# pmgbergen/porepy

Hardware: AMD Instinct MI355X
Metric: cells/sec MPFA assemble+solve, 3D unstructured grid (higher is better)
Workload: dtype f64

## Files before the change

include/porefv.h:

```cpp
#ifndef POREFV_H
#define POREFV_H

#include <stddef.h>
#include <stdint.h>

#ifdef __cplusplus
extern "C" {
#endif

typedef struct pfv_ctx pfv_ctx;

typedef enum {
  PFV_OK = 0,
  PFV_ERR_SINGULAR = 1,
  PFV_ERR_CELL_SHAPE = 2,
  PFV_ERR_HIP = 3,
  PFV_ERR_ARGUMENT = 4,
  PFV_ERR_UNSUPPORTED = 5,
  PFV_ERR_NOT_CONVERGED = 6
} pfv_status;

enum {
  PFV_MAT_FLUX = 0,
  PFV_MAT_BOUND_FLUX = 1,
// ... 401 lines not shown
pfv_status pfv_set_stream(pfv_ctx* h, void* hip_stream);
pfv_status pfv_reset_stream(pfv_ctx* h);
pfv_status pfv_sync(pfv_ctx* h);

pfv_status pfv_get_stats(pfv_ctx* h, pfv_stats* out);
pfv_status pfv_get_stats_n(pfv_ctx* h, void* out, size_t struct_size);

enum { PFV_KERNEL_SPMV_A = 0, PFV_KERNEL_NODE = 1, PFV_KERNEL_FACE = 2,
       PFV_KERNEL_AMG_SMOOTH = 3,
       PFV_KERNEL_TRIAD = 4,
       PFV_KERNEL_READ = 5         };
pfv_status pfv_time_kernel(pfv_ctx* h, int kernel, int reps, double* avg_ms);

pfv_status pfv_debug_copy(pfv_ctx* h, int which, double* dst, int64_t count);

#ifdef __cplusplus
}
#endif
#endif
```

porepy_amd/_lib.py:

```python
from __future__ import annotations

import ctypes as C
import os

import numpy as np

_HERE = os.path.dirname(os.path.abspath(__file__))
DEFAULT_LIBRARY = os.path.join(_HERE, "csrc", "libporefv_hip.so")

MAT_FLUX, MAT_BOUND_FLUX, MAT_BOUND_PRESSURE_CELL, MAT_BOUND_PRESSURE_FACE = 0, 1, 2, 3
MAT_VECTOR_SOURCE, MAT_BOUND_PRESSURE_VECTOR_SOURCE, MAT_SYSTEM = 4, 5, 6
MAT_STRESS, MAT_BOUND_STRESS, MAT_BOUND_DISPLACEMENT_CELL, MAT_BOUND_DISPLACEMENT_FACE, MAT_MECH_SYSTEM = 7, 8, 9, 10, 11
MAT_USER_SYSTEM = 12
MAT_FLUX_JACOBIAN = 13
MAT_UPWIND, MAT_UPWIND_RHS_DIR, MAT_UPWIND_RHS_NEU, MAT_TRANSPORT_SYSTEM = 14, 15, 16, 17
MAT_ADVDIFF_SYSTEM = 18
BC_DIR, BC_NEU, BC_ROB, BC_INTERNAL = 1, 2, 4, 8
SOLVE_CG, SOLVE_BICGSTAB, SOLVE_GMRES = 0, 1, 2
PRECOND_JACOBI, PRECOND_AMG, PRECOND_BLOCK, PRECOND_AMG_NNS, PRECOND_SWEEP = 0, 1, 2, 3, 4
FLUXFN_LINEAR, FLUXFN_COREY, FLUXFN_TABLE = 0, 1, 2
DISCR_REBUILD_TOPOLOGY, DISCR_SKIP_VECTOR_SOURCE = 1, 2

STATUS_NAMES = {
    0: "ok", 1: "singular local system", 2: "unsupported cell shape", 3: "HIP error",
# ... 8 lines not shown
    "pfv_spmv_device_rows", "pfv_copy_device_vector", "pfv_set_stream",
    "pfv_mpsa_set_params", "pfv_mpsa_discretize", "pfv_mpsa_assemble",
    "pfv_mpfa_discretize_faces", "pfv_set_system", "pfv_tpfa_discretize", "pfv_mpsa_discretize_faces", "pfv_set_preconditioner", "pfv_amg_setup", "pfv_amg_setup_sharded", "pfv_amg_apply_device", "pfv_csr_from_host", "pfv_csr_from_matrix", "pfv_csr_block_diag", "pfv_csr_matmul", "pfv_csr_axpby", "pfv_csr_transpose", "pfv_csr_bmat", "pfv_csr_scale", "pfv_csr_divide", "pfv_csr_spmv", "pfv_csr_spmv_device", "pfv_csr_info", "pfv_csr_get", "pfv_csr_set_system", "pfv_csr_free", "pfv_reset_stream", "pfv_mpsa_set_robin", "pfv_mpsa_set_basis", "pfv_mpfa_set_subface_bc", "pfv_mpsa_set_subface_bc", "pfv_mpsa_set_subface_basis",
    "pfv_biot_set_alphas", "pfv_biot_discretize", "pfv_biot_matrix_info", "pfv_biot_get_matrix",
    "pfv_set_vectors_on_device", "pfv_set_periodic", "pfv_biot_discretize_faces", "pfv_solve_sharded", "pfv_tpfa_transmissibility_ad",
    "pfv_get_matrix_rows", "pfv_active_size", "pfv_device_memory",
    "pfv_rccl_unique_id", "pfv_rccl_comm_create", "pfv_rccl_set_halo_plan", "pfv_rccl_hooks", "pfv_rccl_stats",
    "pfv_rccl_last_error", "pfv_rccl_comm_destroy", "pfv_mpfa_ad_flux_system", "pfv_host_alloc", "pfv_host_free",
    "pfv_mpsa_set_subface_eta", "pfv_mpsa_set_reconstruction_eta", "pfv_mpsa_set_reconstruction_eta_subface", "pfv_get_stats_n", "pfv_set_block_preconditioner",
    "pfv_mpfa_set_permeability", "pfv_set_near_null_space", "pfv_amg_nns_level", "pfv_amg_nns_apply_device", "pfv_amg_level",
    "pfv_mpfa_face_flux", "pfv_upwind_set_bc", "pfv_upwind_discretize", "pfv_upwind_assemble", "pfv_transport_advance",
    "pfv_advdiff_assemble", "pfv_advdiff_advance", "pfv_advdiff_face_flux", "pfv_resident_flux",
    "pfv_sweep_info", "pfv_transport_advance_multi", "pfv_transport_advance_nl", "pfv_transport_advance_nl_multi",
    "pfv_transport_advance_react", "pfv_transport_adjoint_multi", "pfv_transport_adjoint_react",
    "pfv_transport_adjoint_nl", "pfv_transport_adjoint_nl_multi", "pfv_flow_adjoint", "pfv_flow_adjoint_exact",
    "pfv_advdiff_adjoint", "pfv_advdiff_adjoint_exact", "pfv_amg_level_rhs",
]


class SolveInfo(C.Structure):
    _fields_ = [("iterations", C.c_int32), ("converged", C.c_int32),
                ("rel_residual", C.c_double), ("solve_ms", C.c_double)]


class Stats(C.Structure):
    _fields_ = [("topology_ms", C.c_double), ("symbolic_ms", C.c_double), ("node_ms", C.c_double),
                ("face_ms", C.c_double), ("assemble_ms", C.c_double), ("solve_ms", C.c_double),
                ("bytes_written_outputs", C.c_double), ("num_nodes", C.c_int64),
                ("num_sub_half_faces", C.c_int64), ("sum_block_sq", C.c_int64),
                ("max_block", C.c_int64), ("amg_setup_ms", C.c_double),
                ("amg_operator_complexity", C.c_double), ("amg_levels", C.c_int64),
# ... 215 lines not shown
    lib.pfv_rccl_last_error.restype = C.c_char_p
    lib.pfv_rccl_comm_destroy.argtypes = [C.c_void_p]
    lib.pfv_rccl_comm_destroy.restype = None
    lib.pfv_device_memory.argtypes = [_h, C.POINTER(C.c_int64), C.POINTER(C.c_int64)]
    lib.pfv_device_memory.restype = C.c_int
    lib.pfv_host_alloc.argtypes = [C.c_size_t, C.POINTER(C.c_void_p)]
    lib.pfv_host_alloc.restype = C.c_int
    lib.pfv_host_free.argtypes = [C.c_void_p]
    lib.pfv_host_free.restype = None
    lib.pfv_active_size.argtypes = [_h, C.POINTER(C.c_int64)]
    lib.pfv_active_size.restype = C.c_int
    lib.pfv_get_matrix_rows.argtypes = [_h, C.c_int, C.c_int64, _ip, _ip, _ip, _dp]
    lib.pfv_get_matrix_rows.restype = C.c_int
    lib.pfv_debug_copy.argtypes = [_h, C.c_int, _dp, C.c_int64]
    lib.pfv_debug_copy.restype = C.c_int
    lib.pfv_spmv_device_rows.argtypes = [_h, C.c_int, C.c_int64, C.c_void_p, C.c_void_p]
    lib.pfv_spmv_device_rows.restype = C.c_int
    lib.pfv_copy_device_vector.argtypes = [_h, C.c_int, C.c_void_p, C.c_int64]
    lib.pfv_copy_device_vector.restype = C.c_int
    lib.pfv_tpfa_transmissibility_ad.argtypes = [_h, _dp, _dp, _dp]
    lib.pfv_tpfa_transmissibility_ad.restype = C.c_int
    lib.pfv_solve_sharded.argtypes = [_h, C.c_int, C.c_double, C.c_int, C.c_int64, C.POINTER(ShardHooks),
                                      C.c_void_p, C.c_void_p, C.POINTER(SolveInfo)]
    lib.pfv_solve_sharded.restype = C.c_int
    lib.pfv_set_stream.argtypes = [_h, C.c_void_p]
    lib.pfv_set_stream.restype = C.c_int
    lib.pfv_mpsa_set_params.argtypes = [_h, _dp, _dp, _up, _up, C.c_double]
    lib.pfv_mpsa_set_params.restype = C.c_int
    lib.pfv_mpsa_discretize.argtypes = [_h, C.c_uint32]
    lib.pfv_mpsa_discretize.restype = C.c_int
# ... 1592 lines not shown
        jac = np.empty((self.ncf, 9), dtype=np.float64)
        self._check(self.lib.pfv_tpfa_transmissibility_ad(self._h, _ptr(K, _dp), _ptr(t, _dp), _ptr(jac, _dp)))
        return t, jac

    def set_stream(self, stream_ptr: int | None):
        self._check(self.lib.pfv_set_stream(self._h, C.c_void_p(stream_ptr or 0)))

    def reset_stream(self):
        self._check(self.lib.pfv_reset_stream(self._h))

    def debug_array(self, which: int, n: int) -> np.ndarray:
        out = np.empty(n, dtype=np.float64)
        self._check(self.lib.pfv_debug_copy(self._h, int(which), _ptr(out, _dp), n))
        return out

    def time_kernel(self, kernel: int, reps: int = 10) -> float:
        ms = C.c_double()
        self._check(self.lib.pfv_time_kernel(self._h, int(kernel), int(reps), C.byref(ms)))
        return ms.value
```

porepy_amd/csrc/backend.h:

```cpp
#pragma once

#include <algorithm>
#include <atomic>
#include <chrono>
#include <cmath>
#include <cstdint>
#include <cstdio>
#include <cstdlib>
#include <cstring>
#include <numeric>
#include <stdexcept>
#include <string>
#include <type_traits>
#include <unordered_map>
#include <vector>

#ifdef PFV_EMULATE
#define PFV_HD
#define PFV_FN inline
#define PFV_LAMBDA [=]
#else
#include <hip/hip_runtime.h>
#include <rocprim/rocprim.hpp>
#define PFV_HD __host__ __device__
// ... 641 lines not shown
    out[i] = acc;
    acc += (TO)in[i];
  }
  out[n] = acc;
#else
  auto it = rocprim::make_transform_iterator(
      rocprim::make_counting_iterator<size_t>(0),
      [in, n] __device__(size_t i) -> TO { return i < n ? (TO)in[i] : TO(0); });
  size_t bytes = 0;
  PFV_HIP_CHECK(rocprim::exclusive_scan(nullptr, bytes, it, out, TO(0), n + 1, rocprim::plus<TO>(), s));
  sc.tmp.ensure(bytes);
  PFV_HIP_CHECK(rocprim::exclusive_scan(sc.tmp.p, bytes, it, out, TO(0), n + 1, rocprim::plus<TO>(), s));
#endif
}

template <class T>
inline T read_scalar(stream_t s, const T* dptr) {
  T v;
  be_d2h(&v, dptr, sizeof(T), s);
  return v;
}

template <class T>
PFV_FN int lower_bound_idx(const T* a, int n, T key) {
  int lo = 0, hi = n;
  while (lo < hi) {
    int mid = (lo + hi) >> 1;
    if (a[mid] < key) lo = mid + 1; else hi = mid;
  }
  return lo;
// ... 49 lines not shown
}
PFV_HD inline int atomic_fetch_add_i32(int* addr, int v) {
#ifdef PFV_EMULATE
  const int old = *addr;
  *addr += v;
  return old;
#else
#if defined(__HIP_DEVICE_COMPILE__)
  return atomicAdd(addr, v);
#else
  (void)addr; (void)v;
  return 0;
#endif
#endif
}
PFV_HD inline void atomic_add_i32(int* addr, int v) {
#ifdef PFV_EMULATE
  *addr += v;
#else
#if defined(__HIP_DEVICE_COMPILE__)
  atomicAdd(addr, v);
#else
  (void)addr; (void)v;
#endif
#endif
}

}
```

porepy_amd/csrc/porefv.hip:

```cpp
#include <cmath>
#include <cstring>

#include "ctx.h"
#include "fluxfn.h"
#include "react.h"
namespace pfv {
static int rccl_exchange_halo(void* user, double* d_x, void* stream);
}
#include "topology.inc"
#include "mpfa_numeric.inc"
#include "linalg.inc"
#include "reorder.inc"
#include "dd.h"
#include "mpsa.inc"
#include "tpfa.inc"
#include "biot.inc"
#include "ad_flux.inc"
#include "upwind.inc"
#include "advdiff.inc"
#include "sweep.inc"
#include "flow_adjoint.inc"
#include "mpfa_adjoint.inc"
#include "advdiff_adjoint.inc"

// ... 4430 lines not shown
      *avg_ms = tm.stop(s) / reps;
    } else {
      require(false, "unknown kernel id");
    }
  });
}

pfv_status pfv_debug_copy(pfv_ctx* h, int which, double* dst, int64_t count) {
  return guarded(h, [&] {
    require(h->have_numeric && dst && count >= 0 && count <= (which == 0 ? h->tab_len : h->tabb_len), "bad argument");
    const double* src = which == 0 ? h->tab.p : h->tabb.p;
    be_d2h(dst, src, sizeof(double) * (size_t)count, h->stream);
  });
}

}

#include "rccl_hooks.inc"
#include "csr_algebra.inc"
```

porepy_amd/csrc/topology.inc:

```

namespace pfv {

static void build_topology(pfv_ctx_impl& c) {
  stream_t s = c.stream;
  const int nd = c.nd;
  const int64_t nc = c.nc, nf = c.nf, nn = c.nn, ncf = c.ncf, nsf = c.nsf;
  const int32_t* cf_ptr = c.cf_ptr;
  const int32_t* cf_idx = c.cf_idx;
  const int8_t* cf_sgn = c.cf_sgn;
  const int32_t* fn_ptr = c.fn_ptr;
  const int32_t* fn_idx = c.fn_idx;

  int bits = 1;
  while ((int64_t(1) << bits) < nn + 1 && bits < 32) ++bits;

  Buf<int32_t> cell_of_e, cnt_e;
  Buf<int64_t> h_off;
  cell_of_e.ensure(ncf);
  cnt_e.ensure(ncf + 1);
  h_off.ensure(ncf + 1);
  {
    int32_t* coe = cell_of_e;
    parallel_for(s, nc, PFV_LAMBDA(int64_t cell) {
      for (int e = cf_ptr[cell]; e < cf_ptr[cell + 1]; ++e) coe[e] = (int32_t)cell;
    });
    int32_t* cnt = cnt_e;
    parallel_for(s, ncf, PFV_LAMBDA(int64_t e) {
      const int f = cf_idx[e];
      cnt[e] = fn_ptr[f + 1] - fn_ptr[f];
    });
  }
  exclusive_scan<int32_t, int64_t>(s, c.scratch, cnt_e.p, h_off.p, (size_t)ncf);
  const int64_t nh = read_scalar<int64_t>(s, h_off.p + ncf);
  if (nh >= (int64_t(1) << 31)) throw Error(5, "more than 2^31 sub-half-faces on one device");
  c.nh = nh;

  Buf<uint32_t> key_in, key_out;
  Buf<int32_t> val_in, val_out;
  key_in.ensure(std::max(nh, nsf));
  key_out.ensure(std::max(nh, nsf));
  val_in.ensure(std::max(nh, nsf));
  val_out.ensure(std::max(nh, nsf));
  {
    uint32_t* k = key_in;
    int32_t* v = val_in;
    const int64_t* off = h_off;
    parallel_for(s, ncf, PFV_LAMBDA(int64_t e) {
      const int f = cf_idx[e];
      const int64_t o = off[e];
      const int a = fn_ptr[f], n = fn_ptr[f + 1] - a;
      for (int i = 0; i < n; ++i) {
        k[o + i] = (uint32_t)fn_idx[a + i];
        v[o + i] = (int32_t)e;
      }
    });
  }
  sort_pairs(s, c.scratch, key_in.p, key_out.p, val_in.p, val_out.p, (size_t)nh, bits);

  c.node_hptr.ensure(nn + 1);
  c.h_cell.ensure(nh);
  c.h_lf.ensure(nh);
  c.h_sgn.ensure(nh);
  c.h_first.ensure(nh);
  Buf<int32_t> h_face;
  h_face.ensure(nh);
  {
    int32_t* hp = c.node_hptr;
    const uint32_t* ks = key_out;
    parallel_for(s, nn + 1, PFV_LAMBDA(int64_t v) {
      hp[v] = lower_bound_idx<uint32_t>(ks, (int)nh, (uint32_t)v);
    });
    int32_t* hc = c.h_cell;
    int32_t* hf = h_face;
    int8_t* hs = c.h_sgn;
    const int32_t* ev = val_out;
    const int32_t* coe = cell_of_e;
    parallel_for(s, nh, PFV_LAMBDA(int64_t h) {
      const int e = ev[h];
      hc[h] = coe[e];
      hf[h] = cf_idx[e];
      hs[h] = cf_sgn[e];
    });
  }
  Buf<uint32_t> h_node;
  h_node.ensure(nh);
  be_d2d(h_node.p, key_out.p, sizeof(uint32_t) * nh, s);

  c.node_fptr.ensure(nn + 1);
  c.node_sf.ensure(nsf);
  c.sf_face.ensure(nsf);
  c.sf_ls.ensure(nsf);
  {
    uint32_t* k = key_in;
    int32_t* v = val_in;
    parallel_for(s, nsf, PFV_LAMBDA(int64_t i) {
      k[i] = (uint32_t)fn_idx[i];
      v[i] = (int32_t)i;
    });
    int32_t* sff = c.sf_face;
    parallel_for(s, nf, PFV_LAMBDA(int64_t f) {
      for (int i = fn_ptr[f]; i < fn_ptr[f + 1]; ++i) sff[i] = (int32_t)f;
    });
  }
  sort_pairs(s, c.scratch, key_in.p, key_out.p, val_in.p, c.node_sf.p, (size_t)nsf, bits);
  {
    Buf<int32_t> mx;
    mx.ensure(2);
    be_memset(mx.p, 0, 2 * sizeof(int32_t), s);
    int32_t* m = mx;
    parallel_for(s, nf, PFV_LAMBDA(int64_t f) { track_max_i32(m, fn_ptr[f + 1] - fn_ptr[f]); });
    parallel_for(s, nc, PFV_LAMBDA(int64_t cell) { track_max_i32(m + 1, cf_ptr[cell + 1] - cf_ptr[cell]); });
    int32_t mxh[2];
    be_d2h(mxh, mx.p, sizeof(mxh), s);
    c.max_face_nodes = mxh[0];
    if (c.max_face_nodes > kMaxFaceNodes)
      throw Error(PFV_ERR_UNSUPPORTED, "faces with more than 8 nodes are not supported");
    c.max_cell_faces = mxh[1];
    if (c.max_cell_faces > kMaxCellFaces)
      throw Error(PFV_ERR_UNSUPPORTED, "cells with more than 16 faces are not supported");
  }
  c.status.ensure(16);
  be_memset(c.status.p, 0, sizeof(int32_t) * 16, s);
  {
    int32_t* fp = c.node_fptr;
    const uint32_t* ks = key_out;
    parallel_for(s, nn + 1, PFV_LAMBDA(int64_t v) {
      fp[v] = lower_bound_idx<uint32_t>(ks, (int)nsf, (uint32_t)v);
    });
    const int32_t* nsf_sorted = c.node_sf;
    uint8_t* ls = c.sf_ls;
    int32_t* st = c.status;
    parallel_for(s, nsf, PFV_LAMBDA(int64_t pos) {
      const int v = (int)ks[pos];
      const int l = (int)pos - fp[v];
      if (l > kMaxBlock) atomic_max_i32(st + 1, l);
      ls[nsf_sorted[pos]] = (uint8_t)(l & 0xff);
    });
  }

  c.face_nsides.ensure(nf);
  Buf<int32_t> face_first;
  face_first.ensure(nf);
  be_memset(c.face_nsides.p, 0, sizeof(int32_t) * nf, s);
  be_memset(face_first.p, 0x7f, sizeof(int32_t) * nf, s);
  {
    int32_t* ns = c.face_nsides;
    int32_t* ff = face_first;
    const int32_t* coe = cell_of_e;
    parallel_for(s, ncf, PFV_LAMBDA(int64_t e) {
      atomic_add_i32(ns + cf_idx[e], 1);
      atomic_min_i32(ff + cf_idx[e], coe[e]);
    });
  }

  Buf<uint8_t> nm_bnd_;
  int32_t* nm_face = c.node_face.ensure(nsf);
  uint8_t* nm_bnd = nm_bnd_.ensure(nsf);
  {
    const int32_t* nsfp = c.node_sf;
    const int32_t* sff = c.sf_face;
    const int32_t* ns = c.face_nsides;
    parallel_for(s, nsf, PFV_LAMBDA(int64_t pos) {
      const int f = sff[nsfp[pos]];
      nm_face[pos] = f;
      nm_bnd[pos] = ns[f] == 1 ? 1 : 0;
    });
  }

  {
    const int32_t* fp = c.node_fptr;
    const int32_t* nsfp = c.node_sf;
    const int32_t* sff = c.sf_face;
    const int32_t* hf = h_face;
    const int32_t* hc = c.h_cell;
    const uint32_t* hn = h_node;
    const int32_t* ff = face_first;
    uint8_t* lf = c.h_lf;
    uint8_t* first = c.h_first;
    int32_t* st = c.status;
    parallel_for(s, nh, PFV_LAMBDA(int64_t h) {
      const int v = (int)hn[h];
      const int a = fp[v], n = fp[v + 1] - a;
      const int f = hf[h];
      int lo = 0, hi = n;
      while (lo < hi) {
        const int mid = (lo + hi) >> 1;
        if (nm_face[a + mid] < f) lo = mid + 1; else hi = mid;
      }
      (void)nsfp; (void)sff;
      if (lo >= n || nm_face[a + lo] != f) atomic_max_i32(st + 0, 1);
      lf[h] = (uint8_t)(lo & 0xff);
      first[h] = (hc[h] == ff[f]) ? 1 : 0;
    });
  }

  c.node_bptr.ensure(nn + 1);
  c.node_tptr.ensure(nn + 1);
  c.node_tbptr.ensure(nn + 1);
  Buf<int32_t> nb_cnt;
  Buf<int64_t> nsq, ntab, ntabb;
  Buf<double> nflop, nflop_scan;
  nb_cnt.ensure(nn + 1);
  nflop.ensure(nn + 1);
  nflop_scan.ensure(nn + 1);
  nsq.ensure(nn + 1);
  ntab.ensure(nn + 1);
  ntabb.ensure(nn + 1);
  {
    const int32_t* hp = c.node_hptr;
    const int32_t* fp = c.node_fptr;
    const int32_t* hc = c.h_cell;
    const int32_t* nsfp = c.node_sf;
    const int32_t* sff = c.sf_face;
    const int32_t* ns = c.face_nsides;
    int32_t* st = c.status;
    int32_t* nbc = nb_cnt;
    int64_t* sq = nsq;
    int64_t* tb = ntab;
    int64_t* tbb = ntabb;
    double* fl = nflop;
    parallel_for(s, nn, PFV_LAMBDA(int64_t v) {
      const int h0 = hp[v], cnt = hp[v + 1] - h0;
      bool ok = (cnt % nd) == 0;
      const int deg = cnt / nd;
      int prev = -1;
      for (int j = 0; ok && j < deg; ++j) {
        const int cc = hc[h0 + nd * j];
        for (int k = 1; k < nd; ++k) ok = ok && (hc[h0 + nd * j + k] == cc);
        ok = ok && (cc > prev);
        prev = cc;
      }
      if (!ok) atomic_max_i32(st + 0, 2);
      const int n = fp[v + 1] - fp[v];
      track_max_i32(st + 1, n);
      track_max_i32(st + 2, deg);
      sq[v] = (int64_t)n * n;
      int nb = 0;
      for (int l = 0; l < n; ++l) nb += nm_bnd[fp[v] + l];
      (void)nsfp; (void)sff; (void)ns;
      nbc[v] = nb;
      track_max_i32(st + 3, nb);
      tb[v] = (int64_t)(n + 1) * ((cnt + 1) & ~1);
      tbb[v] = 2 * (int64_t)n * nb;
      fl[v] = 2.0 * n * n * n + 2.0 * nd * n * cnt + 2.0 * (1 + nd) * n * nb + 60.0 * nd * nd * deg;
    });
  }
  int32_t st_host[4];
  be_d2h(st_host, c.status.p, sizeof(st_host), s);
  if (st_host[0] == 2)
    throw Error(PFV_ERR_CELL_SHAPE,
                "a cell does not have exactly nd faces meeting in one of its nodes (e.g. pyramid)");
  if (st_host[0] == 1) throw Error(PFV_ERR_ARGUMENT, "cell_faces / face_nodes are inconsistent");
  c.max_block = st_host[1];
  c.max_deg = st_host[2];
  c.max_bnd_per_node = st_host[3];
  if (c.max_block > kMaxBlock || c.max_deg > kMaxBlock)
    throw Error(PFV_ERR_UNSUPPORTED, "more than 255 faces or cells meet in one node");
  Buf<int64_t> sq_scan;
  sq_scan.ensure(nn + 1);
  exclusive_scan<int64_t, int64_t>(s, c.scratch, nsq.p, sq_scan.p, (size_t)nn);
  exclusive_scan<double, double>(s, c.scratch, nflop.p, nflop_scan.p, (size_t)nn);
  exclusive_scan<int64_t, int64_t>(s, c.scratch, ntab.p, c.node_tptr.p, (size_t)nn);
  exclusive_scan<int64_t, int64_t>(s, c.scratch, ntabb.p, c.node_tbptr.p, (size_t)nn);
  exclusive_scan<int32_t, int32_t>(s, c.scratch, nb_cnt.p, c.node_bptr.p, (size_t)nn);
  int32_t nb_total = 0;
  {
    Buf<double> tot;
    double* tp = tot.ensure(8);
    const int64_t* sqs = sq_scan;
    const double* fls = nflop_scan;
    const int64_t* tpt = c.node_tptr;
    const int64_t* tbp = c.node_tbptr;
    const int32_t* nbp = c.node_bptr;
    parallel_for(s, 1, PFV_LAMBDA(int64_t) {
      int64_t* ti = reinterpret_cast<int64_t*>(tp);
      ti[0] = sqs[nn];
      tp[1] = fls[nn];
      ti[2] = tpt[nn];
      ti[3] = tbp[nn];
      ti[4] = (int64_t)nbp[nn];
    });
    double th[5];
    be_d2h(th, tp, sizeof(th), s);
    const int64_t* thi = reinterpret_cast<const int64_t*>(th);
    c.sum_block_sq = thi[0];
    c.stats.node_flops = th[1];
    c.tab_len = thi[2];
    c.tabb_len = thi[3];
    nb_total = (int32_t)thi[4];
  }
  c.node_bfaces.ensure(nb_total);
  c.node_bls.ensure(nb_total);
  c.node_cells.ensure(nh / nd + 1);
  {
    const int32_t* fp = c.node_fptr;
    const int32_t* nsfp = c.node_sf;
    const int32_t* sff = c.sf_face;
    const int32_t* ns = c.face_nsides;
    const int32_t* bp = c.node_bptr;
    int32_t* bf = c.node_bfaces;
    uint8_t* bl = c.node_bls;
    parallel_for(s, nn, PFV_LAMBDA(int64_t v) {
      int o = bp[v];
      const int n = fp[v + 1] - fp[v];
      for (int l = 0; l < n; ++l) {
        if (nm_bnd[fp[v] + l]) {
          bf[o] = nm_face[fp[v] + l];
          bl[o] = (uint8_t)l;
          ++o;
        }
      }
      (void)nsfp; (void)sff; (void)ns;
    });
    const int32_t* hc = c.h_cell;
    int32_t* ncl = c.node_cells;
    parallel_for(s, nh / nd, PFV_LAMBDA(int64_t i) { ncl[i] = hc[(int64_t)nd * i]; });
  }

  c.face_order.ensure(nf);
  {
    uint32_t* k = key_in.ensure(nf);
    int32_t* v = val_in.ensure(nf);
    key_out.ensure(nf);
    const double* fc = c.fcen;
    double lo[3], sc[3];
    for (int d = 0; d < 3; ++d) {
      lo[d] = c.bbox_lo[d];
      const double ext = c.bbox_hi[d] - c.bbox_lo[d];
      sc[d] = ext > 0 ? 1023.999 / ext : 0.0;
    }
    const double lo0 = lo[0], lo1 = lo[1], lo2 = lo[2], sc0 = sc[0], sc1 = sc[1], sc2 = sc[2];
    parallel_for(s, nf, PFV_LAMBDA(int64_t f) {
// ... 5 lines not shown
      for (int d = 0; d < 3; ++d) {
        uint32_t x = q[d] & 0x3ffu;
        x = (x | (x << 16)) & 0x030000ffu;
        x = (x | (x << 8)) & 0x0300f00fu;
        x = (x | (x << 4)) & 0x030c30c3u;
        x = (x | (x << 2)) & 0x09249249u;
        code |= x << d;
      }
      k[f] = code;
      v[f] = (int32_t)f;
    });
    sort_pairs(s, c.scratch, key_in.p, key_out.p, val_in.p, c.face_order.p, (size_t)nf, 30);
  }

  {
    const int nclass = kNumClasses;
    Buf<int32_t> bnd_dev;
    bnd_dev.ensure(nclass);
    be_h2d(bnd_dev.p, kClassBounds, sizeof(int) * nclass, s);
    uint32_t* k = key_in.ensure(nn);
    int32_t* v = val_in.ensure(nn);
    key_out.ensure(nn);
    c.node_order.ensure(nn);
    const int32_t* fp = c.node_fptr;
    const int32_t* bd = bnd_dev;
    parallel_for(s, nn, PFV_LAMBDA(int64_t node) {
      const int n = fp[node + 1] - fp[node];
      int cls = 0;
      while (cls < nclass - 1 && n > bd[cls]) ++cls;
      k[node] = (uint32_t)cls;
      v[node] = (int32_t)node;
    });
    sort_pairs(s, c.scratch, key_in.p, key_out.p, val_in.p, c.node_order.p, (size_t)nn, 4);
    Buf<int32_t> cb_dev;
    int32_t* cbd = cb_dev.ensure(nclass + 1);
    const uint32_t* ks = key_out;
    parallel_for(s, nclass + 1, PFV_LAMBDA(int64_t cls) { cbd[cls] = lower_bound_idx<uint32_t>(ks, (int)nn, (uint32_t)cls); });
    std::vector<int32_t> cbh(nclass + 1);
    be_d2h(cbh.data(), cbd, sizeof(int32_t) * (nclass + 1), s);
    c.class_begin.assign(nclass + 1, nn);
    for (int cls = 0; cls <= nclass; ++cls) c.class_begin[cls] = cbh[cls];
  }
  c.have_topology = true;
  c.topo_key = 0;
  c.stats.num_nodes = nn;
  c.stats.num_sub_half_faces = nh;
  c.stats.sum_block_sq = c.sum_block_sq;
  c.stats.max_block = c.max_block;
  c.stats.node_table_doubles = c.tab_len + c.tabb_len;
}

template <class RankT = uint8_t, int EPL = 4>
PFV_FN int merge_unique_lds(const WaveCtx& w, const int32_t* buf, const int32_t* off, int nl,
                            int32_t* merged, unsigned long long* mask, int32_t* out,
                            RankT* rank_out = nullptr) {
  const int m = off[nl];
// ... 792 lines not shown
```

Baseline: 35.12 million.

## Restructure topology build to fuse kernels and batch device-to-host readbacks

Rewrites build_topology so several small kernels are merged. Cell and face max-degree reductions now happen inside the fill kernels, the count array is replaced by a transform-iterator scan, and node pointers are filled inside the half-face kernel. All host readbacks (status, sums, table lengths, class bounds) are packed into one buffer and copied once, instead of through several synchronous transfers. This cuts launches and host-device synchronisations during discretization, at the cost of block reductions with atomics and a more intricate ordering. It also adds a debug API for dumping topology arrays.

```diff
diff --git a/include/porefv.h b/include/porefv.h
--- a/include/porefv.h
+++ b/include/porefv.h
@@ -439,6 +439,9 @@
 
 pfv_status pfv_debug_copy(pfv_ctx* h, int which, double* dst, int64_t count);
 
+enum { PFV_TOPO_SCALARS = 20, PFV_TOPO_NUM_CLASSES = 13 };
+pfv_status pfv_debug_topology(pfv_ctx* h, int which, void* dst, int64_t count);
+
 #ifdef __cplusplus
 }
 #endif
diff --git a/porepy_amd/_lib.py b/porepy_amd/_lib.py
--- a/porepy_amd/_lib.py
+++ b/porepy_amd/_lib.py
@@ -46,7 +46,7 @@
     "pfv_sweep_info", "pfv_transport_advance_multi", "pfv_transport_advance_nl", "pfv_transport_advance_nl_multi",
     "pfv_transport_advance_react", "pfv_transport_adjoint_multi", "pfv_transport_adjoint_react",
     "pfv_transport_adjoint_nl", "pfv_transport_adjoint_nl_multi", "pfv_flow_adjoint", "pfv_flow_adjoint_exact",
-    "pfv_advdiff_adjoint", "pfv_advdiff_adjoint_exact", "pfv_amg_level_rhs",
+    "pfv_advdiff_adjoint", "pfv_advdiff_adjoint_exact", "pfv_amg_level_rhs", "pfv_debug_topology",
 ]
 
 
@@ -292,6 +292,8 @@
     lib.pfv_get_matrix_rows.restype = C.c_int
     lib.pfv_debug_copy.argtypes = [_h, C.c_int, _dp, C.c_int64]
     lib.pfv_debug_copy.restype = C.c_int
+    lib.pfv_debug_topology.argtypes = [_h, C.c_int, C.c_void_p, C.c_int64]
+    lib.pfv_debug_topology.restype = C.c_int
     lib.pfv_spmv_device_rows.argtypes = [_h, C.c_int, C.c_int64, C.c_void_p, C.c_void_p]
     lib.pfv_spmv_device_rows.restype = C.c_int
     lib.pfv_copy_device_vector.argtypes = [_h, C.c_int, C.c_void_p, C.c_int64]
@@ -1914,6 +1916,35 @@
         self._check(self.lib.pfv_debug_copy(self._h, int(which), _ptr(out, _dp), n))
         return out
 
+    TOPOLOGY_ARRAYS = {
+        "node_hptr": (0, np.int32, lambda c, t: c.nn + 1), "h_cell": (1, np.int32, lambda c, t: t["nh"]),
+        "h_lf": (2, np.uint8, lambda c, t: t["nh"]), "h_sgn": (3, np.int8, lambda c, t: t["nh"]),
+        "h_first": (4, np.uint8, lambda c, t: t["nh"]), "node_fptr": (5, np.int32, lambda c, t: c.nn + 1),
+        "node_sf": (6, np.int32, lambda c, t: c.nsf), "sf_face": (7, np.int32, lambda c, t: c.nsf),
+        "sf_ls": (8, np.uint8, lambda c, t: c.nsf), "node_face": (9, np.int32, lambda c, t: c.nsf),
+        "face_nsides": (10, np.int32, lambda c, t: c.nf), "node_bptr": (11, np.int32, lambda c, t: c.nn + 1),
+        "node_bfaces": (12, np.int32, lambda c, t: t["nb_total"]), "node_bls": (13, np.uint8, lambda c, t: t["nb_total"]),
+        "node_cells": (14, np.int32, lambda c, t: t["nh"] // c.nd), "node_tptr": (15, np.int64, lambda c, t: c.nn + 1),
+        "node_tbptr": (16, np.int64, lambda c, t: c.nn + 1), "face_order": (17, np.int32, lambda c, t: c.nf),
+        "node_order": (18, np.int32, lambda c, t: c.nn), "class_begin": (19, np.int64, lambda c, t: 14),
+    }
+    TOPOLOGY_SCALARS = ("nh", "max_face_nodes", "max_cell_faces", "max_block", "max_deg", "max_bnd_per_node",
+                        "sum_block_sq", "tab_len", "tabb_len", "nb_total")
+
+    def topology_scalars(self) -> dict:
+        out = np.empty(len(self.TOPOLOGY_SCALARS), dtype=np.int64)
+        self._check(self.lib.pfv_debug_topology(self._h, 20, out.ctypes.data_as(C.c_void_p), out.size))
+        return dict(zip(self.TOPOLOGY_SCALARS, (int(v) for v in out)))
+
+    def topology_array(self, name: str):
+        sc = self.topology_scalars()
+        if name in sc:
+            return sc[name]
+        which, dtype, size = self.TOPOLOGY_ARRAYS[name]
+        out = np.empty(int(size(self, sc)), dtype=dtype)
+        self._check(self.lib.pfv_debug_topology(self._h, which, out.ctypes.data_as(C.c_void_p), out.size))
+        return out
+
     def time_kernel(self, kernel: int, reps: int = 10) -> float:
         ms = C.c_double()
         self._check(self.lib.pfv_time_kernel(self._h, int(kernel), int(reps), C.byref(ms)))
diff --git a/porepy_amd/csrc/backend.h b/porepy_amd/csrc/backend.h
--- a/porepy_amd/csrc/backend.h
+++ b/porepy_amd/csrc/backend.h
@@ -679,6 +679,27 @@
 #endif
 }
 
+template <class TO, class F>
+inline void exclusive_scan_of(stream_t s, Scratch& sc, F f, TO* out, size_t n) {
+#ifdef PFV_EMULATE
+  (void)s; (void)sc;
+  TO acc = 0;
+  for (size_t i = 0; i < n; ++i) {
+    out[i] = acc;
+    acc += (TO)f(i);
+  }
+  out[n] = acc;
+#else
+  auto it = rocprim::make_transform_iterator(
+      rocprim::make_counting_iterator<size_t>(0),
+      [f, n] __device__(size_t i) -> TO { return i < n ? (TO)f(i) : TO(0); });
+  size_t bytes = 0;
+  PFV_HIP_CHECK(rocprim::exclusive_scan(nullptr, bytes, it, out, TO(0), n + 1, rocprim::plus<TO>(), s));
+  sc.tmp.ensure(bytes);
+  PFV_HIP_CHECK(rocprim::exclusive_scan(sc.tmp.p, bytes, it, out, TO(0), n + 1, rocprim::plus<TO>(), s));
+#endif
+}
+
 template <class T>
 inline T read_scalar(stream_t s, const T* dptr) {
   T v;
@@ -758,7 +779,7 @@
 #endif
 #endif
 }
-PFV_HD inline void atomic_add_i32(int* addr, int v) {
+PFV_HD inline void atomic_add_u64(unsigned long long* addr, unsigned long long v) {
 #ifdef PFV_EMULATE
   *addr += v;
 #else
@@ -769,5 +790,27 @@
 #endif
 #endif
 }
-
-}
+PFV_HD inline void atomic_add_f64(double* addr, double v) {
+#ifdef PFV_EMULATE
+  *addr += v;
+#else
+#if defined(__HIP_DEVICE_COMPILE__)
+  atomicAdd(addr, v);
+#else
+  (void)addr; (void)v;
+#endif
+#endif
+}
+PFV_HD inline void atomic_add_i32(int* addr, int v) {
+#ifdef PFV_EMULATE
+  *addr += v;
+#else
+#if defined(__HIP_DEVICE_COMPILE__)
+  atomicAdd(addr, v);
+#else
+  (void)addr; (void)v;
+#endif
+#endif
+}
+
+}
diff --git a/porepy_amd/csrc/porefv.hip b/porepy_amd/csrc/porefv.hip
--- a/porepy_amd/csrc/porefv.hip
+++ b/porepy_amd/csrc/porefv.hip
@@ -4468,6 +4468,37 @@
   });
 }
 
+pfv_status pfv_debug_topology(pfv_ctx* h, int which, void* dst, int64_t count) {
+  return guarded(h, [&] {
+    require(h->have_topology && dst && count >= 0, "bad argument (discretize first)");
+    static_assert(PFV_TOPO_NUM_CLASSES == pfv::kNumClasses, "header out of step with the size classes");
+    const int64_t nn = h->nn, nf = h->nf, nsf = h->nsf, nh = h->nh;
+    const int64_t nb = pfv::read_scalar<int32_t>(h->stream, h->node_bptr.p + nn);
+    if (which == PFV_TOPO_SCALARS) {
+      require(count == 10, "ten scalars");
+      const int64_t v[10] = {nh, h->max_face_nodes, h->max_cell_faces, h->max_block, h->max_deg,
+                             h->max_bnd_per_node, h->sum_block_sq, h->tab_len, h->tabb_len, nb};
+      std::memcpy(dst, v, sizeof(v));
+      return;
+    }
+    if (which == 19) {
+      require(count == (int64_t)h->class_begin.size(), "class_begin has kNumClasses + 1 entries");
+      std::memcpy(dst, h->class_begin.data(), sizeof(int64_t) * (size_t)count);
+      return;
+    }
+    struct Arr { const void* p; size_t elem; int64_t n; };
+    const Arr arrs[19] = {
+        {h->node_hptr.p, 4, nn + 1}, {h->h_cell.p, 4, nh},      {h->h_lf.p, 1, nh},          {h->h_sgn.p, 1, nh},
+        {h->h_first.p, 1, nh},       {h->node_fptr.p, 4, nn + 1}, {h->node_sf.p, 4, nsf},    {h->sf_face.p, 4, nsf},
+        {h->sf_ls.p, 1, nsf},        {h->node_face.p, 4, nsf},  {h->face_nsides.p, 4, nf},   {h->node_bptr.p, 4, nn + 1},
+        {h->node_bfaces.p, 4, nb},   {h->node_bls.p, 1, nb},    {h->node_cells.p, 4, nh / h->nd},
+        {h->node_tptr.p, 8, nn + 1}, {h->node_tbptr.p, 8, nn + 1}, {h->face_order.p, 4, nf}, {h->node_order.p, 4, nn}};
+    require(which >= 0 && which < 19, "unknown topology array");
+    require(count == arrs[which].n, "count is not the array's size");
+    be_d2h(dst, arrs[which].p, arrs[which].elem * (size_t)count, h->stream);
+  });
+}
+
 }
 
 #include "rccl_hooks.inc"
diff --git a/porepy_amd/csrc/topology.inc b/porepy_amd/csrc/topology.inc
--- a/porepy_amd/csrc/topology.inc
+++ b/porepy_amd/csrc/topology.inc
@@ -1,5 +1,30 @@
 
 namespace pfv {
+
+template <class T>
+PFV_FN T block_max(const WaveCtx& w, T* sh, T v) {
+  sh[w.lane] = v;
+  w.sync();
+  for (int o = w.width >> 1; o > 0; o >>= 1) {
+    if (w.lane < o && sh[w.lane + o] > sh[w.lane]) sh[w.lane] = sh[w.lane + o];
+    w.sync();
+  }
+  const T r = sh[0];
+  w.sync();
+  return r;
+}
+template <class T>
+PFV_FN T block_sum(const WaveCtx& w, T* sh, T v) {
+  sh[w.lane] = v;
+  w.sync();
+  for (int o = w.width >> 1; o > 0; o >>= 1) {
+    if (w.lane < o) sh[w.lane] += sh[w.lane + o];
+    w.sync();
+  }
+  const T r = sh[0];
+  w.sync();
+  return r;
+}
 
 static void build_topology(pfv_ctx_impl& c) {
   stream_t s = c.stream;
@@ -14,33 +39,132 @@
   int bits = 1;
   while ((int64_t(1) << bits) < nn + 1 && bits < 32) ++bits;
 
-  Buf<int32_t> cell_of_e, cnt_e;
+  Buf<int32_t> cell_of_e;
   Buf<int64_t> h_off;
   cell_of_e.ensure(ncf);
-  cnt_e.ensure(ncf + 1);
-  h_off.ensure(ncf + 1);
+  h_off.ensure(ncf + 2);
+  int32_t* mx = reinterpret_cast<int32_t*>(h_off.p + ncf + 1);
+  be_memset(mx, 0, 2 * sizeof(int32_t), s);
+  c.sf_face.ensure(nsf);
+  Buf<int32_t> sf_id;
+  sf_id.ensure(nsf);
   {
     int32_t* coe = cell_of_e;
-    parallel_for(s, nc, PFV_LAMBDA(int64_t cell) {
-      for (int e = cf_ptr[cell]; e < cf_ptr[cell + 1]; ++e) coe[e] = (int32_t)cell;
-    });
-    int32_t* cnt = cnt_e;
+    const int nbc = (int)std::min<int64_t>(2048, (nc + 255) / 256);
+    block_for<256>(s, nbc, 256 * sizeof(int32_t), PFV_LAMBDA(const WaveCtx& w) {
+      int32_t* sh = reinterpret_cast<int32_t*>(w.lds);
+      const int64_t lo = nc * w.item / nbc, hi = nc * (w.item + 1) / nbc;
+      int m = 0;
+      for (int64_t cell = lo + w.lane; cell < hi; cell += w.width) {
+        const int a = cf_ptr[cell], b = cf_ptr[cell + 1];
+        m = b - a > m ? b - a : m;
+        for (int e = a; e < b; ++e) coe[e] = (int32_t)cell;
+      }
+      m = block_max(w, sh, m);
+      if (w.lane0() && m > 0) atomic_max_i32(mx + 1, m);
+    });
+    int32_t* sff = c.sf_face;
+    int32_t* v = sf_id;
+    const int nbf = (int)std::min<int64_t>(2048, (nf + 255) / 256);
+    block_for<256>(s, nbf, 256 * sizeof(int32_t), PFV_LAMBDA(const WaveCtx& w) {
+      int32_t* sh = reinterpret_cast<int32_t*>(w.lds);
+      const int64_t lo = nf * w.item / nbf, hi = nf * (w.item + 1) / nbf;
+      int m = 0;
+      for (int64_t f = lo + w.lane; f < hi; f += w.width) {
+        const int a = fn_ptr[f], b = fn_ptr[f + 1];
+        m = b - a > m ? b - a : m;
+        for (int i = a; i < b; ++i) {
+          sff[i] = (int32_t)f;
+          v[i] = (int32_t)i;
+        }
+      }
+      m = block_max(w, sh, m);
+      if (w.lane0() && m > 0) atomic_max_i32(mx + 0, m);
+    });
+  }
+  exclusive_scan_of<int64_t>(s, c.scratch, PFV_LAMBDA(size_t e) {
+    const int f = cf_idx[e];
+    return (int64_t)(fn_ptr[f + 1] - fn_ptr[f]);
+  }, h_off.p, (size_t)ncf);
+
+  c.node_fptr.ensure(nn + 1);
+  c.node_sf.ensure(nsf);
+  c.sf_ls.ensure(nsf);
+  c.status.ensure(16);
+  be_memset(c.status.p, 0, sizeof(int32_t) * 16, s);
+  c.face_nsides.ensure(nf);
+  Buf<int32_t> face_first;
+  face_first.ensure(nf);
+  be_memset(c.face_nsides.p, 0, sizeof(int32_t) * nf, s);
+  be_memset(face_first.p, 0x7f, sizeof(int32_t) * nf, s);
+  {
+    int32_t* ns = c.face_nsides;
+    int32_t* ff = face_first;
+    const int32_t* coe = cell_of_e;
     parallel_for(s, ncf, PFV_LAMBDA(int64_t e) {
-      const int f = cf_idx[e];
-      cnt[e] = fn_ptr[f + 1] - fn_ptr[f];
-    });
-  }
-  exclusive_scan<int32_t, int64_t>(s, c.scratch, cnt_e.p, h_off.p, (size_t)ncf);
-  const int64_t nh = read_scalar<int64_t>(s, h_off.p + ncf);
+      atomic_add_i32(ns + cf_idx[e], 1);
+      atomic_min_i32(ff + cf_idx[e], coe[e]);
+    });
+  }
+  Buf<uint8_t> nm_bnd_;
+  int32_t* nm_face = c.node_face.ensure(nsf);
+  uint8_t* nm_bnd = nm_bnd_.ensure(nsf);
+  Buf<int32_t> nb_cnt;
+  nb_cnt.ensure(nn + 1);
+  be_memset(nb_cnt.p, 0, sizeof(int32_t) * (nn + 1), s);
+  {
+    Buf<uint32_t> sf_node;
+    sf_node.ensure(nsf);
+    sort_pairs(s, c.scratch, reinterpret_cast<const uint32_t*>(fn_idx), sf_node.p, sf_id.p, c.node_sf.p, (size_t)nsf, bits);
+    int32_t* fp = c.node_fptr;
+    const uint32_t* ks = sf_node;
+    parallel_for(s, nn + 1, PFV_LAMBDA(int64_t v) {
+      fp[v] = lower_bound_idx<uint32_t>(ks, (int)nsf, (uint32_t)v);
+    });
+    const int32_t* nsf_sorted = c.node_sf;
+    const int32_t* sff = c.sf_face;
+    const int32_t* ns = c.face_nsides;
+    uint8_t* ls = c.sf_ls;
+    int32_t* st = c.status;
+    int32_t* nbc = nb_cnt;
+    parallel_for(s, nsf, PFV_LAMBDA(int64_t pos) {
+      const int v = (int)ks[pos];
+      const int l = (int)pos - fp[v];
+      if (l > kMaxBlock) atomic_max_i32(st + 1, l);
+      const int i = nsf_sorted[pos];
+      ls[i] = (uint8_t)(l & 0xff);
+      const int f = sff[i];
+      const bool bnd = ns[f] == 1;
+      nm_face[pos] = f;
+      nm_bnd[pos] = bnd ? 1 : 0;
+      if (bnd && v < nn) atomic_add_i32(nbc + v, 1);
+    });
+  }
+  sf_id.release();
+
+  int64_t head[2];
+  be_d2h(head, h_off.p + ncf, sizeof(head), s);
+  const int64_t nh = head[0];
   if (nh >= (int64_t(1) << 31)) throw Error(5, "more than 2^31 sub-half-faces on one device");
   c.nh = nh;
+  {
+    int32_t mxh[2];
+    std::memcpy(mxh, &head[1], sizeof(mxh));
+    c.max_face_nodes = mxh[0];
+    if (c.max_face_nodes > kMaxFaceNodes)
+      throw Error(PFV_ERR_UNSUPPORTED, "faces with more than 8 nodes are not supported");
+    c.max_cell_faces = mxh[1];
+    if (c.max_cell_faces > kMaxCellFaces)
+      throw Error(PFV_ERR_UNSUPPORTED, "cells with more than 16 faces are not supported");
+  }
 
   Buf<uint32_t> key_in, key_out;
   Buf<int32_t> val_in, val_out;
-  key_in.ensure(std::max(nh, nsf));
-  key_out.ensure(std::max(nh, nsf));
-  val_in.ensure(std::max(nh, nsf));
-  val_out.ensure(std::max(nh, nsf));
+  const int64_t nkey = std::max(std::max(nh, nf), nn);
+  key_in.ensure(nkey);
+  key_out.ensure(nkey);
+  val_in.ensure(nkey);
+  val_out.ensure(nh);
   {
     uint32_t* k = key_in;
     int32_t* v = val_in;
@@ -62,260 +186,108 @@
   c.h_lf.ensure(nh);
   c.h_sgn.ensure(nh);
   c.h_first.ensure(nh);
-  Buf<int32_t> h_face;
-  h_face.ensure(nh);
   {
     int32_t* hp = c.node_hptr;
     const uint32_t* ks = key_out;
-    parallel_for(s, nn + 1, PFV_LAMBDA(int64_t v) {
-      hp[v] = lower_bound_idx<uint32_t>(ks, (int)nh, (uint32_t)v);
-    });
+    if (nh == 0) be_memset(hp, 0, sizeof(int32_t) * (nn + 1), s);
     int32_t* hc = c.h_cell;
-    int32_t* hf = h_face;
     int8_t* hs = c.h_sgn;
+    uint8_t* lf = c.h_lf;
+    uint8_t* first = c.h_first;
     const int32_t* ev = val_out;
     const int32_t* coe = cell_of_e;
+    const int32_t* ff = face_first;
+    const uint8_t* ls = c.sf_ls;
+    int32_t* st = c.status;
     parallel_for(s, nh, PFV_LAMBDA(int64_t h) {
       const int e = ev[h];
-      hc[h] = coe[e];
-      hf[h] = cf_idx[e];
+      const int v = (int)ks[h];
+      const int vp = h > 0 ? (int)ks[h - 1] : -1;
+      for (int u = vp + 1; u <= v && u <= nn; ++u) hp[u] = (int32_t)h;
+      if (h == nh - 1)
+        for (int64_t u = (int64_t)v + 1; u <= nn; ++u) hp[u] = (int32_t)nh;
+      const int f = cf_idx[e];
+      const int cell = coe[e];
+      const int a = fn_ptr[f], n = fn_ptr[f + 1] - a;
+      int i = 0;
+      while (i < n && fn_idx[a + i] != v) ++i;
+      if (i >= n) atomic_max_i32(st + 0, 1);
+      hc[h] = cell;
       hs[h] = cf_sgn[e];
-    });
-  }
-  Buf<uint32_t> h_node;
-  h_node.ensure(nh);
-  be_d2d(h_node.p, key_out.p, sizeof(uint32_t) * nh, s);
-
-  c.node_fptr.ensure(nn + 1);
-  c.node_sf.ensure(nsf);
-  c.sf_face.ensure(nsf);
-  c.sf_ls.ensure(nsf);
-  {
-    uint32_t* k = key_in;
-    int32_t* v = val_in;
-    parallel_for(s, nsf, PFV_LAMBDA(int64_t i) {
-      k[i] = (uint32_t)fn_idx[i];
-      v[i] = (int32_t)i;
-    });
-    int32_t* sff = c.sf_face;
-    parallel_for(s, nf, PFV_LAMBDA(int64_t f) {
-      for (int i = fn_ptr[f]; i < fn_ptr[f + 1]; ++i) sff[i] = (int32_t)f;
-    });
-  }
-  sort_pairs(s, c.scratch, key_in.p, key_out.p, val_in.p, c.node_sf.p, (size_t)nsf, bits);
-  {
-    Buf<int32_t> mx;
-    mx.ensure(2);
-    be_memset(mx.p, 0, 2 * sizeof(int32_t), s);
-    int32_t* m = mx;
-    parallel_for(s, nf, PFV_LAMBDA(int64_t f) { track_max_i32(m, fn_ptr[f + 1] - fn_ptr[f]); });
-    parallel_for(s, nc, PFV_LAMBDA(int64_t cell) { track_max_i32(m + 1, cf_ptr[cell + 1] - cf_ptr[cell]); });
-    int32_t mxh[2];
-    be_d2h(mxh, mx.p, sizeof(mxh), s);
-    c.max_face_nodes = mxh[0];
-    if (c.max_face_nodes > kMaxFaceNodes)
-      throw Error(PFV_ERR_UNSUPPORTED, "faces with more than 8 nodes are not supported");
-    c.max_cell_faces = mxh[1];
-    if (c.max_cell_faces > kMaxCellFaces)
-      throw Error(PFV_ERR_UNSUPPORTED, "cells with more than 16 faces are not supported");
-  }
-  c.status.ensure(16);
-  be_memset(c.status.p, 0, sizeof(int32_t) * 16, s);
-  {
-    int32_t* fp = c.node_fptr;
-    const uint32_t* ks = key_out;
-    parallel_for(s, nn + 1, PFV_LAMBDA(int64_t v) {
-      fp[v] = lower_bound_idx<uint32_t>(ks, (int)nsf, (uint32_t)v);
-    });
-    const int32_t* nsf_sorted = c.node_sf;
-    uint8_t* ls = c.sf_ls;
-    int32_t* st = c.status;
-    parallel_for(s, nsf, PFV_LAMBDA(int64_t pos) {
-      const int v = (int)ks[pos];
-      const int l = (int)pos - fp[v];
-      if (l > kMaxBlock) atomic_max_i32(st + 1, l);
-      ls[nsf_sorted[pos]] = (uint8_t)(l & 0xff);
-    });
-  }
-
-  c.face_nsides.ensure(nf);
-  Buf<int32_t> face_first;
-  face_first.ensure(nf);
-  be_memset(c.face_nsides.p, 0, sizeof(int32_t) * nf, s);
-  be_memset(face_first.p, 0x7f, sizeof(int32_t) * nf, s);
-  {
-    int32_t* ns = c.face_nsides;
-    int32_t* ff = face_first;
-    const int32_t* coe = cell_of_e;
-    parallel_for(s, ncf, PFV_LAMBDA(int64_t e) {
-      atomic_add_i32(ns + cf_idx[e], 1);
-      atomic_min_i32(ff + cf_idx[e], coe[e]);
-    });
-  }
-
-  Buf<uint8_t> nm_bnd_;
-  int32_t* nm_face = c.node_face.ensure(nsf);
-  uint8_t* nm_bnd = nm_bnd_.ensure(nsf);
-  {
-    const int32_t* nsfp = c.node_sf;
-    const int32_t* sff = c.sf_face;
-    const int32_t* ns = c.face_nsides;
-    parallel_for(s, nsf, PFV_LAMBDA(int64_t pos) {
-      const int f = sff[nsfp[pos]];
-      nm_face[pos] = f;
-      nm_bnd[pos] = ns[f] == 1 ? 1 : 0;
-    });
-  }
-
-  {
-    const int32_t* fp = c.node_fptr;
-    const int32_t* nsfp = c.node_sf;
-    const int32_t* sff = c.sf_face;
-    const int32_t* hf = h_face;
-    const int32_t* hc = c.h_cell;
-    const uint32_t* hn = h_node;
-    const int32_t* ff = face_first;
-    uint8_t* lf = c.h_lf;
-    uint8_t* first = c.h_first;
-    int32_t* st = c.status;
-    parallel_for(s, nh, PFV_LAMBDA(int64_t h) {
-      const int v = (int)hn[h];
-      const int a = fp[v], n = fp[v + 1] - a;
-      const int f = hf[h];
-      int lo = 0, hi = n;
-      while (lo < hi) {
-        const int mid = (lo + hi) >> 1;
-        if (nm_face[a + mid] < f) lo = mid + 1; else hi = mid;
-      }
-      (void)nsfp; (void)sff;
-      if (lo >= n || nm_face[a + lo] != f) atomic_max_i32(st + 0, 1);
-      lf[h] = (uint8_t)(lo & 0xff);
-      first[h] = (hc[h] == ff[f]) ? 1 : 0;
+      lf[h] = i < n ? ls[a + i] : (uint8_t)0;
+      first[h] = (cell == ff[f]) ? 1 : 0;
     });
   }
 
   c.node_bptr.ensure(nn + 1);
   c.node_tptr.ensure(nn + 1);
   c.node_tbptr.ensure(nn + 1);
-  Buf<int32_t> nb_cnt;
-  Buf<int64_t> nsq, ntab, ntabb;
-  Buf<double> nflop, nflop_scan;
-  nb_cnt.ensure(nn + 1);
-  nflop.ensure(nn + 1);
-  nflop_scan.ensure(nn + 1);
-  nsq.ensure(nn + 1);
+  c.node_cells.ensure(nh / nd + 1);
+  Buf<int64_t> ntab, ntabb;
   ntab.ensure(nn + 1);
   ntabb.ensure(nn + 1);
+  const int nclass = kNumClasses;
+  Buf<int64_t> pack_;
+  int64_t* pack = pack_.ensure(10 + nclass);
+  be_memset(pack, 0, sizeof(int64_t) * (10 + nclass), s);
   {
     const int32_t* hp = c.node_hptr;
     const int32_t* fp = c.node_fptr;
     const int32_t* hc = c.h_cell;
-    const int32_t* nsfp = c.node_sf;
-    const int32_t* sff = c.sf_face;
-    const int32_t* ns = c.face_nsides;
+    int32_t* ncl = c.node_cells;
     int32_t* st = c.status;
-    int32_t* nbc = nb_cnt;
-    int64_t* sq = nsq;
+    const int32_t* nbc = nb_cnt;
     int64_t* tb = ntab;
     int64_t* tbb = ntabb;
-    double* fl = nflop;
-    parallel_for(s, nn, PFV_LAMBDA(int64_t v) {
-      const int h0 = hp[v], cnt = hp[v + 1] - h0;
-      bool ok = (cnt % nd) == 0;
-      const int deg = cnt / nd;
-      int prev = -1;
-      for (int j = 0; ok && j < deg; ++j) {
-        const int cc = hc[h0 + nd * j];
-        for (int k = 1; k < nd; ++k) ok = ok && (hc[h0 + nd * j + k] == cc);
-        ok = ok && (cc > prev);
-        prev = cc;
-      }
-      if (!ok) atomic_max_i32(st + 0, 2);
-      const int n = fp[v + 1] - fp[v];
-      track_max_i32(st + 1, n);
-      track_max_i32(st + 2, deg);
-      sq[v] = (int64_t)n * n;
-      int nb = 0;
-      for (int l = 0; l < n; ++l) nb += nm_bnd[fp[v] + l];
-      (void)nsfp; (void)sff; (void)ns;
-      nbc[v] = nb;
-      track_max_i32(st + 3, nb);
-      tb[v] = (int64_t)(n + 1) * ((cnt + 1) & ~1);
-      tbb[v] = 2 * (int64_t)n * nb;
-      fl[v] = 2.0 * n * n * n + 2.0 * nd * n * cnt + 2.0 * (1 + nd) * n * nb + 60.0 * nd * nd * deg;
-    });
-  }
-  int32_t st_host[4];
-  be_d2h(st_host, c.status.p, sizeof(st_host), s);
-  if (st_host[0] == 2)
-    throw Error(PFV_ERR_CELL_SHAPE,
-                "a cell does not have exactly nd faces meeting in one of its nodes (e.g. pyramid)");
-  if (st_host[0] == 1) throw Error(PFV_ERR_ARGUMENT, "cell_faces / face_nodes are inconsistent");
-  c.max_block = st_host[1];
-  c.max_deg = st_host[2];
-  c.max_bnd_per_node = st_host[3];
-  if (c.max_block > kMaxBlock || c.max_deg > kMaxBlock)
-    throw Error(PFV_ERR_UNSUPPORTED, "more than 255 faces or cells meet in one node");
-  Buf<int64_t> sq_scan;
-  sq_scan.ensure(nn + 1);
-  exclusive_scan<int64_t, int64_t>(s, c.scratch, nsq.p, sq_scan.p, (size_t)nn);
-  exclusive_scan<double, double>(s, c.scratch, nflop.p, nflop_scan.p, (size_t)nn);
+    const int nbn = (int)std::min<int64_t>(2048, (nn + 15) / 16);
+    block_for<256>(s, nbn, 256 * sizeof(double), PFV_LAMBDA(const WaveCtx& w) {
+      int32_t* shi = reinterpret_cast<int32_t*>(w.lds);
+      const int G = w.width >= 16 ? 16 : 1;
+      const int ng = w.width / G, g = w.lane / G, sl = w.lane % G;
+      const int64_t lo = nn * w.item / nbn, hi = nn * (w.item + 1) / nbn;
+      int mn = 0, mdeg = 0, mnb = 0;
+      int64_t ssq = 0;
+      double sfl = 0.0;
+      for (int64_t v = lo + g; v < hi; v += ng) {
+        const int h0 = hp[v], cnt = hp[v + 1] - h0;
+        const int deg = cnt / nd;
+        bool bad = (cnt % nd) != 0;
+        for (int j = sl; j < deg; j += G) {
+          const int cc = hc[h0 + nd * j];
+          for (int k = 1; k < nd; ++k) bad = bad || hc[h0 + nd * j + k] != cc;
+          if (j > 0) bad = bad || !(cc > hc[h0 + nd * (j - 1)]);
+          ncl[h0 / nd + j] = cc;
+        }
+        if (bad) atomic_max_i32(st + 0, 2);
+        if (sl == 0) {
+          const int n = fp[v + 1] - fp[v];
+          const int nb = nbc[v];
+          mn = n > mn ? n : mn;
+          mdeg = deg > mdeg ? deg : mdeg;
+          mnb = nb > mnb ? nb : mnb;
+          tb[v] = (int64_t)(n + 1) * ((cnt + 1) & ~1);
+          tbb[v] = 2 * (int64_t)n * nb;
+          ssq += (int64_t)n * n;
+          sfl += 2.0 * n * n * n + 2.0 * nd * n * cnt + 2.0 * (1 + nd) * n * nb + 60.0 * nd * nd * deg;
+        }
+      }
+      mn = block_max(w, shi, mn);
+      mdeg = block_max(w, shi, mdeg);
+      mnb = block_max(w, shi, mnb);
+      ssq = block_sum(w, reinterpret_cast<int64_t*>(w.lds), ssq);
+      sfl = block_sum(w, reinterpret_cast<double*>(w.lds), sfl);
+      if (w.lane0()) {
+        if (mn > 0) atomic_max_i32(st + 1, mn);
+        if (mdeg > 0) atomic_max_i32(st + 2, mdeg);
+        if (mnb > 0) atomic_max_i32(st + 3, mnb);
+        atomic_add_u64(reinterpret_cast<unsigned long long*>(pack + 4), (unsigned long long)ssq);
+        atomic_add_f64(reinterpret_cast<double*>(pack + 5), sfl);
+      }
+    });
+  }
   exclusive_scan<int64_t, int64_t>(s, c.scratch, ntab.p, c.node_tptr.p, (size_t)nn);
   exclusive_scan<int64_t, int64_t>(s, c.scratch, ntabb.p, c.node_tbptr.p, (size_t)nn);
   exclusive_scan<int32_t, int32_t>(s, c.scratch, nb_cnt.p, c.node_bptr.p, (size_t)nn);
-  int32_t nb_total = 0;
-  {
-    Buf<double> tot;
-    double* tp = tot.ensure(8);
-    const int64_t* sqs = sq_scan;
-    const double* fls = nflop_scan;
-    const int64_t* tpt = c.node_tptr;
-    const int64_t* tbp = c.node_tbptr;
-    const int32_t* nbp = c.node_bptr;
-    parallel_for(s, 1, PFV_LAMBDA(int64_t) {
-      int64_t* ti = reinterpret_cast<int64_t*>(tp);
-      ti[0] = sqs[nn];
-      tp[1] = fls[nn];
-      ti[2] = tpt[nn];
-      ti[3] = tbp[nn];
-      ti[4] = (int64_t)nbp[nn];
-    });
-    double th[5];
-    be_d2h(th, tp, sizeof(th), s);
-    const int64_t* thi = reinterpret_cast<const int64_t*>(th);
-    c.sum_block_sq = thi[0];
-    c.stats.node_flops = th[1];
-    c.tab_len = thi[2];
-    c.tabb_len = thi[3];
-    nb_total = (int32_t)thi[4];
-  }
-  c.node_bfaces.ensure(nb_total);
-  c.node_bls.ensure(nb_total);
-  c.node_cells.ensure(nh / nd + 1);
-  {
-    const int32_t* fp = c.node_fptr;
-    const int32_t* nsfp = c.node_sf;
-    const int32_t* sff = c.sf_face;
-    const int32_t* ns = c.face_nsides;
-    const int32_t* bp = c.node_bptr;
-    int32_t* bf = c.node_bfaces;
-    uint8_t* bl = c.node_bls;
-    parallel_for(s, nn, PFV_LAMBDA(int64_t v) {
-      int o = bp[v];
-      const int n = fp[v + 1] - fp[v];
-      for (int l = 0; l < n; ++l) {
-        if (nm_bnd[fp[v] + l]) {
-          bf[o] = nm_face[fp[v] + l];
-          bl[o] = (uint8_t)l;
-          ++o;
-        }
-      }
-      (void)nsfp; (void)sff; (void)ns;
-    });
-    const int32_t* hc = c.h_cell;
-    int32_t* ncl = c.node_cells;
-    parallel_for(s, nh / nd, PFV_LAMBDA(int64_t i) { ncl[i] = hc[(int64_t)nd * i]; });
-  }
 
   c.face_order.ensure(nf);
   {
@@ -351,32 +323,74 @@
   }
 
   {
-    const int nclass = kNumClasses;
-    Buf<int32_t> bnd_dev;
-    bnd_dev.ensure(nclass);
-    be_h2d(bnd_dev.p, kClassBounds, sizeof(int) * nclass, s);
+    struct { int b[kNumClasses]; } bd;
+    for (int i = 0; i < nclass; ++i) bd.b[i] = kClassBounds[i];
     uint32_t* k = key_in.ensure(nn);
     int32_t* v = val_in.ensure(nn);
     key_out.ensure(nn);
     c.node_order.ensure(nn);
     const int32_t* fp = c.node_fptr;
-    const int32_t* bd = bnd_dev;
     parallel_for(s, nn, PFV_LAMBDA(int64_t node) {
       const int n = fp[node + 1] - fp[node];
       int cls = 0;
-      while (cls < nclass - 1 && n > bd[cls]) ++cls;
+      for (int i = 0; i < kNumClasses - 1; ++i) cls += n > bd.b[i] ? 1 : 0;
       k[node] = (uint32_t)cls;
       v[node] = (int32_t)node;
     });
     sort_pairs(s, c.scratch, key_in.p, key_out.p, val_in.p, c.node_order.p, (size_t)nn, 4);
-    Buf<int32_t> cb_dev;
-    int32_t* cbd = cb_dev.ensure(nclass + 1);
     const uint32_t* ks = key_out;
-    parallel_for(s, nclass + 1, PFV_LAMBDA(int64_t cls) { cbd[cls] = lower_bound_idx<uint32_t>(ks, (int)nn, (uint32_t)cls); });
-    std::vector<int32_t> cbh(nclass + 1);
-    be_d2h(cbh.data(), cbd, sizeof(int32_t) * (nclass + 1), s);
-    c.class_begin.assign(nclass + 1, nn);
-    for (int cls = 0; cls <= nclass; ++cls) c.class_begin[cls] = cbh[cls];
+    const int32_t* st = c.status;
+    const int64_t* tpt = c.node_tptr;
+    const int64_t* tbp = c.node_tbptr;
+    const int32_t* nbp = c.node_bptr;
+    parallel_for(s, nclass + 1, PFV_LAMBDA(int64_t cls) {
+      pack[9 + cls] = lower_bound_idx<uint32_t>(ks, (int)nn, (uint32_t)cls);
+      if (cls == 0) {
+        for (int i = 0; i < 4; ++i) pack[i] = st[i];
+        pack[6] = tpt[nn];
+        pack[7] = tbp[nn];
+        pack[8] = (int64_t)nbp[nn];
+      }
+    });
+  }
+
+  std::vector<int64_t> ph(10 + nclass);
+  be_d2h(ph.data(), pack, sizeof(int64_t) * (10 + nclass), s);
+  if (ph[0] == 2)
+    throw Error(PFV_ERR_CELL_SHAPE,
+                "a cell does not have exactly nd faces meeting in one of its nodes (e.g. pyramid)");
+  if (ph[0] == 1) throw Error(PFV_ERR_ARGUMENT, "cell_faces / face_nodes are inconsistent");
+  c.max_block = (int)ph[1];
+  c.max_deg = (int)ph[2];
+  c.max_bnd_per_node = (int)ph[3];
+  if (c.max_block > kMaxBlock || c.max_deg > kMaxBlock)
+    throw Error(PFV_ERR_UNSUPPORTED, "more than 255 faces or cells meet in one node");
+  c.sum_block_sq = ph[4];
+  std::memcpy(&c.stats.node_flops, &ph[5], sizeof(double));
+  c.tab_len = ph[6];
+  c.tabb_len = ph[7];
+  const int32_t nb_total = (int32_t)ph[8];
+  c.class_begin.assign(nclass + 1, nn);
+  for (int cls = 0; cls <= nclass; ++cls) c.class_begin[cls] = ph[9 + cls];
+
+  c.node_bfaces.ensure(nb_total);
+  c.node_bls.ensure(nb_total);
+  {
+    const int32_t* fp = c.node_fptr;
+    const int32_t* bp = c.node_bptr;
+    int32_t* bf = c.node_bfaces;
+    uint8_t* bl = c.node_bls;
+    parallel_for(s, nn, PFV_LAMBDA(int64_t v) {
+      int o = bp[v];
+      const int n = fp[v + 1] - fp[v];
+      for (int l = 0; l < n; ++l) {
+        if (nm_bnd[fp[v] + l]) {
+          bf[o] = nm_face[fp[v] + l];
+          bl[o] = (uint8_t)l;
+          ++o;
+        }
+      }
+    });
   }
   c.have_topology = true;
   c.topo_key = 0;
```

Result: no change. 35.41 million (median of 6 runs) (+0.8%).
